# consensus-shipyard/ipc-filecoin-proofs

Hardware: AMD Instinct MI355X
Metric: Merkle proofs verified/sec + HBM GB/s, 1M-receipt synthetic tipset, 1/2/4/8 GPU (higher is better)
Workload: dtype u64; 1 GPU; BASELINE.json configs[2] (the 1M-receipt tipset the metric is quoted on): 1000000 receipts (Amtv0<Receipt> + one Amt<...; receipts_per_gpu=1000000, claims_per_gpu=1000000, witness_blocks_per_gpu=1288038, witness_bytes_per_gpu=439923915, scan_matches=1002, device=AMD Radeon Graphics

## Files before the change

ipc-filecoin-proofs_amd/csrc/kernels/verify_dev.h:

```cpp
#pragma once
#include "claims_dev.h"
#include "event_table.h"
#include "amt_enum.h"
#include "event_table.h"
#include "tipset_ctx.h"
#include "types_dev.h"

namespace ipcfp {


constexpr unsigned long long kEmptySlot64 = ~0ULL;

__device__ __forceinline__ uint32_t exec_find(const unsigned long long* slots, uint32_t mask, const CidKey* keys,
                                              const CidKey& key) {
    const uint64_t h = cid_hash64(key);
    uint32_t s = uint32_t(h >> 32) & mask;
    for (;;) {
        const unsigned long long cur = slots[s];
        if (cur == kEmptySlot64) return kNoBlock;
        if (uint32_t(cur >> 32) == uint32_t(h) && cid_equal(keys[uint32_t(cur)], key)) return uint32_t(cur);
        s = (s + 1) & mask;
    }
}

__device__ __forceinline__ bool ev_trusted(const ipcfp_trust_policy_t& t, long long epoch) {
    if (t.kind == 0) return true;
    if (t.ec_chain_empty) return false;
    return epoch >= t.min_epoch && epoch <= t.max_epoch;
}

__device__ __forceinline__ bool bytes_equal_global(const uint8_t* __restrict__ a, const uint8_t* __restrict__ b, uint32_t n) {
    uint64_t diff = 0;
    uint32_t i = 0;
    typedef unsigned long long u64x2_t __attribute__((ext_vector_type(2)));
    for (; i + 16 <= n; i += 16) {
        u64x2_t x, y;
        __builtin_memcpy(&x, a + i, 16);
        __builtin_memcpy(&y, b + i, 16);
        diff |= (x.x ^ y.x) | (x.y ^ y.y);
    }
    for (; i + 8 <= n; i += 8) {
        uint64_t x, y;
        __builtin_memcpy(&x, a + i, 8);
        __builtin_memcpy(&y, b + i, 8);
        diff |= x ^ y;
    }
    for (; i < n; ++i) diff |= uint64_t(a[i] ^ b[i]);
    return diff == 0;
}

__device__ __forceinline__ uint32_t verify_event_record(const WitnessView& w, const EventClaimPacked& c, const EventRec& e,
                                                        const uint8_t* __restrict__ blob, const ipcfp_event_filter_t& filter,
                                                        bool has_filter) {
    if (e.emitter != c.emitter) return IPCFP_ST_FALSE_EMITTER;
    if (!(e.base_flags & kEvIsLog)) return IPCFP_ST_FALSE_NOT_EVM_LOG;
    const uint32_t nt = uint32_t(e.base_flags >> kEvTopicShift) & 0xffu;
    if (nt != c.n_topics) return IPCFP_ST_FALSE_TOPIC_COUNT;
    const uint8_t* item = w.arena + (e.base_flags & kEvBaseMask);
    const bool case_a = (e.base_flags & kEvCaseA) != 0;
    for (uint32_t i = 0; i < nt; ++i) {
        const uint8_t* claimed = blob + c.topics_off + 33u * i;
        if (!claimed[0]) return IPCFP_ST_FALSE_TOPIC;
        const uint32_t rel = case_a ? uint32_t(e.topic_rel[0]) + 32u * i : uint32_t(e.topic_rel[i & 3u]);
        if (!bytes_equal_global(item + rel, claimed + 1, 32)) return IPCFP_ST_FALSE_TOPIC;
    }
    if (!(c.flags & EC_DATA_MATCHABLE) || c.data_len != e.data_len) return IPCFP_ST_FALSE_DATA;
    if (!bytes_equal_global(item + e.data_rel, blob + c.data_off, c.data_len)) return IPCFP_ST_FALSE_DATA;
    if (has_filter) {
        if (nt < 2) return IPCFP_ST_FALSE_FILTER;
        const uint32_t r1 = case_a ? uint32_t(e.topic_rel[0]) + 32u : uint32_t(e.topic_rel[1]);
        if (!bytes_equal_global(item + e.topic_rel[0], filter.topic0, 32) || !bytes_equal_global(item + r1, filter.topic1, 32))
            return IPCFP_ST_FALSE_FILTER;
    }
    return IPCFP_ST_TRUE;
}

__device__ __forceinline__ uint32_t verify_event_prefix(const EventClaimPacked& c, const TipsetCtxDev& tc,
                                                        const ipcfp_trust_policy_t& trust) {
    if (!(tc.flags & TC_PARENTS_PARSED) || !(tc.flags & TC_CHILD_PARSED)) return IPCFP_ST_ERR_BAD_CLAIM;
    if (!ev_trusted(trust, c.parent_epoch)) return IPCFP_ST_FALSE_UNTRUSTED_PARENT;
    if (!ev_trusted(trust, c.child_epoch)) return IPCFP_ST_FALSE_UNTRUSTED_CHILD;
    if (tc.child_status != IPCFP_ST_TRUE) return tc.child_status;
    if (!tc.parents_match) return IPCFP_ST_FALSE_PARENTS_MISMATCH;
    if (tc.child_height != c.child_epoch) return IPCFP_ST_FALSE_CHILD_EPOCH;
    if (tc.n_parents == 0) return IPCFP_ST_ERR_EMPTY_PARENTS;
    if (tc.parent0_status != IPCFP_ST_TRUE) return tc.parent0_status;
    if (tc.parent0_height != c.parent_epoch) return IPCFP_ST_FALSE_PARENT_EPOCH;
    if (tc.exec_status != IPCFP_ST_TRUE) return tc.exec_status;
    if (!(c.flags & EC_MSG_PARSED)) return IPCFP_ST_ERR_BAD_CLAIM;
    if (tc.exec_inv && c.exec_index < tc.exec_len && cid_equal(tc.exec_keys[tc.exec_inv[c.exec_index]], c.message))
        return IPCFP_ST_TRUE;
    const uint32_t raw = tc.exec_slots ? exec_find(tc.exec_slots, tc.exec_mask, tc.exec_keys, c.message) : kNoBlock;
    if (raw == kNoBlock) return IPCFP_ST_FALSE_MSG_NOT_IN_EXEC;
    if (uint64_t(tc.exec_pos[raw]) != c.exec_index) return IPCFP_ST_FALSE_EXEC_INDEX;
    return IPCFP_ST_TRUE;
}

struct EventCtxFacts {
    uint32_t flags, n_parents, child_status, parents_match, parent0_status, exec_status;
    long long child_height, parent0_height;
    const CidKey* exec_keys;
    const uint32_t* exec_inv;
    uint64_t exec_len;
    bool has_receipt_table;
    uint64_t n_receipt_leaves, receipt_first;
    const ReceiptRec* receipt_recs;
    const EventRec* event_recs;
};

__device__ __forceinline__ EventCtxFacts event_ctx_facts(const TipsetCtxDev& tc) {
    return EventCtxFacts{tc.flags,        tc.n_parents,      tc.child_status, tc.parents_match,
                         tc.parent0_status, tc.exec_status,  tc.child_height, tc.parent0_height,
                         tc.exec_keys,    tc.exec_inv,       tc.exec_len,     tc.receipt_leaves != nullptr && tc.receipt_recs != nullptr,
                         tc.n_receipt_leaves, tc.receipt_first, tc.receipt_recs, tc.event_recs};
}

struct Verdict {
    uint32_t st = IPCFP_ST_TRUE;
    bool settled = false;
    __device__ __forceinline__ void rung(bool fails, uint32_t status) {
        st = (!settled && fails) ? status : st;
        settled = settled || fails;
    }
};

__device__ __forceinline__ void event_prefix_rungs(Verdict& v, const EventClaimPacked& c, const EventCtxFacts& f,
                                                   const ipcfp_trust_policy_t& trust) {
    v.rung(!(f.flags & TC_PARENTS_PARSED) || !(f.flags & TC_CHILD_PARSED), IPCFP_ST_ERR_BAD_CLAIM);
    v.rung(!ev_trusted(trust, c.parent_epoch), IPCFP_ST_FALSE_UNTRUSTED_PARENT);
    v.rung(!ev_trusted(trust, c.child_epoch), IPCFP_ST_FALSE_UNTRUSTED_CHILD);
    v.rung(f.child_status != IPCFP_ST_TRUE, f.child_status);
    v.rung(!f.parents_match, IPCFP_ST_FALSE_PARENTS_MISMATCH);
    v.rung(f.child_height != c.child_epoch, IPCFP_ST_FALSE_CHILD_EPOCH);
    v.rung(f.n_parents == 0, IPCFP_ST_ERR_EMPTY_PARENTS);
    v.rung(f.parent0_status != IPCFP_ST_TRUE, f.parent0_status);
    v.rung(f.parent0_height != c.parent_epoch, IPCFP_ST_FALSE_PARENT_EPOCH);
    v.rung(f.exec_status != IPCFP_ST_TRUE, f.exec_status);
    v.rung(!(c.flags & EC_MSG_PARSED), IPCFP_ST_ERR_BAD_CLAIM);
}

__device__ __forceinline__ uint32_t verify_event_from_table(const WitnessView& w, const EventClaimPacked& c,
                                                            const TipsetCtxDev& tc, const uint8_t* __restrict__ blob,
                                                            const ipcfp_event_filter_t& filter, bool has_filter,
                                                            ValueLoc* where, bool& settled) {
    settled = false;
    if (!tc.receipt_leaves || !tc.receipt_recs || c.exec_index < tc.receipt_first ||
        c.exec_index - tc.receipt_first >= tc.n_receipt_leaves)
        return kStPending;
    const ReceiptRec rr = tc.receipt_recs[c.exec_index - tc.receipt_first];
    if (rr.kind == RK_WALK) return kStPending;
    settled = true;
    if (rr.kind == RK_NO_EVENTS) return IPCFP_ST_FALSE_NO_EVENTS_ROOT;
    if (rr.kind >= 64) return rr.kind;
    if (c.event_index == ~0ULL) return IPCFP_ST_ERR;
    if (c.event_index >= 64 || !((rr.bitmap >> c.event_index) & 1ull)) return IPCFP_ST_FALSE_NO_EVENT;
    const EventRec e = tc.event_recs[rr.first + __popcll(rr.bitmap & ((1ull << c.event_index) - 1ull))];
    if (where) *where = ValueLoc{rr.block, uint32_t((e.base_flags & kEvBaseMask) - w.off[rr.block]), e.ev_len};
    return verify_event_record(w, c, e, blob, filter, has_filter);
}

__device__ __forceinline__ bool claim_in_bounds(const EventClaimPacked& c, uint32_t n_ctxs, uint64_t blob_len) {
    return c.context < n_ctxs && c.n_topics <= (1u << 20) && uint64_t(c.topics_off) + 33ull * c.n_topics <= blob_len &&
           uint64_t(c.data_off) + c.data_len <= blob_len;
}

}
```

ipc-filecoin-proofs_amd/csrc/kernels/verify_table.hip:

```cpp
#include <hip/hip_runtime.h>

#include <cstddef>

#include "../common.h"
#include "launch.h"
#include "verify_dev.h"

namespace ipcfp {

typedef unsigned long long u64x2_t __attribute__((ext_vector_type(2)));

__device__ __forceinline__ u64x2_t ld16(const uint8_t* __restrict__ p) {
    u64x2_t v;
    __builtin_memcpy(&v, p, 16);
    return v;
}
__device__ __forceinline__ bool differ32(const u64x2_t a[2], const u64x2_t b[2]) {
    return (((a[0].x ^ b[0].x) | (a[0].y ^ b[0].y)) | ((a[1].x ^ b[1].x) | (a[1].y ^ b[1].y))) != 0;
}

struct ClaimedBytes {
    u64x2_t topic[2][2];
    uint32_t flag[2];
    u64x2_t data[2];
};

__device__ __forceinline__ void load_claimed(const EventClaimPacked& c, const uint8_t* __restrict__ blob, ClaimedBytes& p) {
    p = ClaimedBytes{};
    if (c.n_topics >= 1 && c.n_topics <= 2) {
        const uint8_t* q = blob + c.topics_off;
        p.flag[0] = q[0];
        p.topic[0][0] = ld16(q + 1);
        p.topic[0][1] = ld16(q + 17);
        if (c.n_topics == 2) {
            p.flag[1] = q[33];
            p.topic[1][0] = ld16(q + 34);
            p.topic[1][1] = ld16(q + 50);
        }
    }
    if ((c.flags & EC_DATA_MATCHABLE) && c.data_len == 32) {
        p.data[0] = ld16(blob + c.data_off);
        p.data[1] = ld16(blob + c.data_off + 16);
    }
}

__device__ __forceinline__ uint32_t verify_event_record_batched(const WitnessView& w, const EventClaimPacked& c, const EventRec& e,
                                                                const ClaimedBytes& p, const uint8_t* __restrict__ blob,
                                                                const ipcfp_event_filter_t& filter, bool has_filter) {
    if (e.emitter != c.emitter) return IPCFP_ST_FALSE_EMITTER;
    if (!(e.base_flags & kEvIsLog)) return IPCFP_ST_FALSE_NOT_EVM_LOG;
    const uint32_t nt = uint32_t(e.base_flags >> kEvTopicShift) & 0xffu;
    if (nt != c.n_topics) return IPCFP_ST_FALSE_TOPIC_COUNT;
    if (nt > 2) return verify_event_record(w, c, e, blob, filter, has_filter);
    const uint8_t* item = w.arena + (e.base_flags & kEvBaseMask);
    const bool case_a = (e.base_flags & kEvCaseA) != 0;
    const uint32_t rel0 = e.topic_rel[0], rel1 = case_a ? uint32_t(e.topic_rel[0]) + 32u : uint32_t(e.topic_rel[1]);
    const bool data_shape = (c.flags & EC_DATA_MATCHABLE) && c.data_len == e.data_len;
    const bool data_batched = data_shape && c.data_len == 32;
    u64x2_t t0[2] = {}, t1[2] = {}, d[2] = {};
    if (nt >= 1) {
        t0[0] = ld16(item + rel0);
        t0[1] = ld16(item + rel0 + 16);
    }
    if (nt == 2) {
        t1[0] = ld16(item + rel1);
        t1[1] = ld16(item + rel1 + 16);
    }
    if (data_batched) {
        d[0] = ld16(item + e.data_rel);
        d[1] = ld16(item + e.data_rel + 16);
    }
    if (nt >= 1 && (!p.flag[0] || differ32(p.topic[0], t0))) return IPCFP_ST_FALSE_TOPIC;
    if (nt == 2 && (!p.flag[1] || differ32(p.topic[1], t1))) return IPCFP_ST_FALSE_TOPIC;
    if (!data_shape) return IPCFP_ST_FALSE_DATA;
    if (data_batched ? differ32(p.data, d) : !bytes_equal_global(item + e.data_rel, blob + c.data_off, c.data_len))
        return IPCFP_ST_FALSE_DATA;
    if (has_filter) {
        if (nt < 2) return IPCFP_ST_FALSE_FILTER;
        u64x2_t f0[2], f1[2];
        __builtin_memcpy(f0, filter.topic0, 32);
        __builtin_memcpy(f1, filter.topic1, 32);
        if (differ32(t0, f0) || differ32(t1, f1)) return IPCFP_ST_FALSE_FILTER;
    }
    return IPCFP_ST_TRUE;
}

__device__ __forceinline__ uint32_t verify_table_one(const WitnessView& w, const EventClaimPacked& c, const TipsetCtxDev& tc,
                                                     const uint8_t* __restrict__ blob, const ipcfp_trust_policy_t& trust,
                                                     const ipcfp_event_filter_t& filter, bool has_filter, ValueLoc* where) {
    ClaimedBytes p;
    load_claimed(c, blob, p);
    const bool tabulated = tc.receipt_leaves && tc.receipt_recs && c.exec_index >= tc.receipt_first &&
                           c.exec_index - tc.receipt_first < tc.n_receipt_leaves;
    ReceiptRec rr{RK_WALK, 0, 0, kNoBlock, 0};
    if (tabulated) rr = tc.receipt_recs[c.exec_index - tc.receipt_first];
    const uint32_t st = verify_event_prefix(c, tc, trust);
    if (st != IPCFP_ST_TRUE) return st;
    if (!tabulated || rr.kind == RK_WALK) return kStPending;
    if (rr.kind == RK_NO_EVENTS) return IPCFP_ST_FALSE_NO_EVENTS_ROOT;
    if (rr.kind >= 64) return rr.kind;
    if (c.event_index == ~0ULL) return IPCFP_ST_ERR;
    if (c.event_index >= 64 || !((rr.bitmap >> c.event_index) & 1ull)) return IPCFP_ST_FALSE_NO_EVENT;
    const EventRec e = tc.event_recs[rr.first + __popcll(rr.bitmap & ((1ull << c.event_index) - 1ull))];
    if (where) *where = ValueLoc{rr.block, uint32_t((e.base_flags & kEvBaseMask) - w.off[rr.block]), e.ev_len};
    return verify_event_record_batched(w, c, e, p, blob, filter, has_filter);
}

typedef const __attribute__((address_space(1))) uint8_t* gbytes_t;
__device__ __forceinline__ gbytes_t guarded(bool ok, const void* p, const void* safe) {
    return ok ? (gbytes_t)p : (gbytes_t)safe;
}
__device__ __forceinline__ u64x2_t ld16(gbytes_t p) {
    u64x2_t v;
    __builtin_memcpy(&v, p, 16);
    return v;
}
__device__ __forceinline__ void batch_end(uint64_t a, uint64_t b = 0, uint64_t c = 0, uint64_t d = 0, uint64_t e = 0) {
    asm volatile("" ::"v"(a), "v"(b), "v"(c), "v"(d), "v"(e));
}

static_assert(offsetof(ReceiptRec, first) == 4 && offsetof(ReceiptRec, bitmap) == 8 && offsetof(ReceiptRec, block) == 16,
              "verify_table_hot reads a ReceiptRec as three words");
static_assert(offsetof(EventRec, topic_rel) == 16 && offsetof(EventRec, data_rel) == 24 && offsetof(EventRec, ev_len) == 26 &&
                  offsetof(EventRec, data_len) == 28,
              "verify_table_hot reads an EventRec as four words");

__device__ __forceinline__ bool hot_shape(const EventClaimPacked& c) {
    return c.n_topics <= 2 && (!(c.flags & EC_DATA_MATCHABLE) || c.data_len == 32);
}

__device__ __forceinline__ uint32_t verify_table_hot(const WitnessView& w, const EventClaimPacked& c, const TipsetCtxDev& tc,
                                                     const uint8_t* __restrict__ blob, const ipcfp_trust_policy_t& trust,
                                                     const ipcfp_event_filter_t& filter, bool has_filter, bool want_where,
                                                     const void* safe, ValueLoc& loc, bool& cold) {
    const EventCtxFacts f = event_ctx_facts(tc);
    Verdict v;
    event_prefix_rungs(v, c, f, trust);
    const bool pre_ok = !v.settled;
    const bool tabulated = f.has_receipt_table && c.exec_index >= f.receipt_first && c.exec_index - f.receipt_first < f.n_receipt_leaves;
    uint64_t rw[3];
    __builtin_memcpy(rw, guarded(tabulated, f.receipt_recs + (c.exec_index - f.receipt_first), safe), 24);
    const bool inv_ok = pre_ok && f.exec_inv && f.exec_keys && c.exec_index < f.exec_len;
    uint32_t inv;
    __builtin_memcpy(&inv, guarded(inv_ok, f.exec_inv + c.exec_index, safe), 4);
    const bool matchable = (c.flags & EC_DATA_MATCHABLE) != 0;
    const gbytes_t q0 = guarded(c.n_topics >= 1, blob + c.topics_off, safe);
    const gbytes_t q1 = guarded(c.n_topics == 2, blob + c.topics_off + 33, safe);
    const gbytes_t qd = guarded(matchable, blob + c.data_off, safe);
    ClaimedBytes p;
    p.flag[0] = q0[0];
    p.topic[0][0] = ld16(q0 + 1);
    p.topic[0][1] = ld16(q0 + 17);
    p.flag[1] = q1[0];
    p.topic[1][0] = ld16(q1 + 1);
    p.topic[1][1] = ld16(q1 + 17);
    p.data[0] = ld16(qd);
    p.data[1] = ld16(qd + 16);
    batch_end(rw[0], rw[1], rw[2], inv);
    const uint32_t rr_kind = uint32_t(rw[0]), rr_first = uint32_t(rw[0] >> 32), rr_block = uint32_t(rw[2]);
    const uint64_t rr_bitmap = rw[1];

    CidKey key;
    __builtin_memcpy(&key, guarded(inv_ok, f.exec_keys + inv, safe), 40);
    const uint32_t bit = uint32_t(c.event_index) & 63u;
    const bool present = c.event_index < 64 && ((rr_bitmap >> bit) & 1ull);
    const bool have_event = pre_ok && tabulated && rr_kind == RK_TABLE && f.event_recs && present;
    const uint32_t slot = rr_first + uint32_t(__popcll(rr_bitmap & ((1ull << bit) - 1ull)));
    uint64_t ew[4];
    __builtin_memcpy(ew, guarded(have_event, f.event_recs + slot, safe), 32);
    uint64_t block_off;
    __builtin_memcpy(&block_off, guarded(want_where && have_event, w.off + rr_block, safe), 8);
    batch_end(key.w[0], key.w[1], key.w[2], key.w[3], key.w[4]);
    batch_end(ew[0], ew[1], ew[2], ew[3], block_off);

    const bool exec_ok = inv_ok && cid_equal(key, c.message);
    v.rung(!tabulated || rr_kind == RK_WALK, kStPending);
    v.rung(rr_kind == RK_NO_EVENTS, IPCFP_ST_FALSE_NO_EVENTS_ROOT);
    v.rung(rr_kind >= 64, rr_kind);
    v.rung(c.event_index == ~0ULL, IPCFP_ST_ERR);
    v.rung(!present, IPCFP_ST_FALSE_NO_EVENT);
    const bool reached = !v.settled;
    cold = pre_ok && (!exec_ok || (reached && !have_event));

    const uint64_t base_flags = ew[0], e_emitter = ew[1];
    const uint32_t rel0 = uint32_t(ew[2]) & 0xffffu, rel1_b = uint32_t(ew[2] >> 16) & 0xffffu;
    const uint32_t data_rel = uint32_t(ew[3]) & 0xffffu, ev_len = uint32_t(ew[3] >> 16) & 0xffffu, e_data_len = uint32_t(ew[3] >> 32);
    v.rung(e_emitter != c.emitter, IPCFP_ST_FALSE_EMITTER);
    v.rung(!(base_flags & kEvIsLog), IPCFP_ST_FALSE_NOT_EVM_LOG);
    const uint32_t nt = uint32_t(base_flags >> kEvTopicShift) & 0xffu;
    v.rung(nt != c.n_topics, IPCFP_ST_FALSE_TOPIC_COUNT);

    const bool bytes_wanted = have_event && exec_ok && !v.settled;
    const uint8_t* item = w.arena + (base_flags & kEvBaseMask);
    const uint32_t rel1 = (base_flags & kEvCaseA) ? rel0 + 32u : rel1_b;
    const bool data_shape = matchable && c.data_len == e_data_len;
    const gbytes_t a0 = guarded(bytes_wanted && nt >= 1, item + rel0, safe);
    const gbytes_t a1 = guarded(bytes_wanted && nt == 2, item + rel1, safe);
    const gbytes_t ad = guarded(bytes_wanted && data_shape, item + data_rel, safe);
    const u64x2_t t0[2] = {ld16(a0), ld16(a0 + 16)}, t1[2] = {ld16(a1), ld16(a1 + 16)}, d[2] = {ld16(ad), ld16(ad + 16)};

    v.rung(nt >= 1 && (!p.flag[0] || differ32(p.topic[0], t0)), IPCFP_ST_FALSE_TOPIC);
    v.rung(nt == 2 && (!p.flag[1] || differ32(p.topic[1], t1)), IPCFP_ST_FALSE_TOPIC);
    v.rung(!data_shape, IPCFP_ST_FALSE_DATA);
    v.rung(differ32(p.data, d), IPCFP_ST_FALSE_DATA);
    u64x2_t f0[2], f1[2];
    __builtin_memcpy(f0, filter.topic0, 32);
    __builtin_memcpy(f1, filter.topic1, 32);
    v.rung(has_filter && nt < 2, IPCFP_ST_FALSE_FILTER);
    v.rung(has_filter && (differ32(t0, f0) || differ32(t1, f1)), IPCFP_ST_FALSE_FILTER);

    const bool located = reached && have_event;
    loc.block = located ? rr_block : kNoBlock;
    loc.off = located ? uint32_t((base_flags & kEvBaseMask) - block_off) : 0u;
    loc.len = located ? ev_len : 0u;
    return v.st;
}

__global__ __launch_bounds__(256) void k_verify_events_table(WitnessView w, const EventClaimPacked* __restrict__ claims, uint32_t n,
                                                             const TipsetCtxDev* __restrict__ ctxs, uint32_t n_ctxs,
                                                             const uint8_t* __restrict__ blob, uint64_t blob_len,
                                                             ipcfp_trust_policy_t trust, ipcfp_event_filter_t filter,
                                                             int has_filter, uint8_t* __restrict__ status,
                                                             ValueLoc* __restrict__ where) {
    const uint32_t t = blockIdx.x * blockDim.x + threadIdx.x;
    const bool live = t < n;
    EventClaimPacked c;
    if (live) c = claims[t];
    else c.context = 0;
    ValueLoc loc{kNoBlock, 0, 0};
    uint32_t st = IPCFP_ST_ERR_BAD_CLAIM;
    const bool inb = live && claim_in_bounds(c, n_ctxs, blob_len);
    const uint32_t ctx0 = __builtin_amdgcn_readfirstlane(inb ? c.context : 0xffffffffu);
    bool cold = inb;
    if (ctx0 != 0xffffffffu && __all(!inb || c.context == ctx0)) {
        if (inb && hot_shape(c)) {
            ValueLoc hot_loc;
            bool again;
            const uint32_t hot_st = verify_table_hot(w, c, ctxs[ctx0], blob, trust, filter, has_filter != 0, where != nullptr,
                                                     claims + t, hot_loc, again);
            st = again ? st : hot_st;
            loc.block = again ? loc.block : hot_loc.block;
            loc.off = again ? loc.off : hot_loc.off;
            loc.len = again ? loc.len : hot_loc.len;
            cold = again;
        }
    }
    if (__any(cold)) {
        if (cold) {
            const EventClaimPacked* mine = claims + t;
            asm volatile("" : "+v"(mine));
            const EventClaimPacked cc = *mine;
            ValueLoc cold_loc{kNoBlock, 0, 0};
            st = verify_table_one(w, cc, ctxs[cc.context], blob, trust, filter, has_filter != 0, &cold_loc);
            loc = cold_loc;
        }
    }
    if (!live) return;
    status[t] = uint8_t(st);
    if (where) where[t] = loc;
}

int launch_verify_events_table(ipcfp_ctx* ctx, const WitnessView& w, const EventClaimPacked* claims_d, uint32_t n,
                               const TipsetCtxDev* ctxs_d, uint32_t n_ctxs, const uint8_t* blob_d, uint64_t blob_len,
                               const ipcfp_trust_policy_t& trust, const ipcfp_event_filter_t& filter, int has_filter,
                               uint8_t* status_d, void* where_d) {
    if (n == 0) return IPCFP_OK;
    hipLaunchKernelGGL(k_verify_events_table, dim3(div_up(n, 256)), dim3(256), 0, ctx->stream, w, claims_d, n, ctxs_d, n_ctxs,
                       blob_d, blob_len, trust, filter, has_filter, status_d, static_cast<ValueLoc*>(where_d));
    IPCFP_HIP(ctx, hipGetLastError());
    return IPCFP_OK;
}

}
```

Baseline: 1.268 billion proofs/s.

## Stage claims and claimed blob window through LDS with coalesced wave-wide copies

The table-verify kernel now copies each wave's claim structs into a per-wave shared-memory region with coalesced 16-byte loads. It then computes the wave's min/max span of claimed topic/data bytes in the blob and stages that window into LDS before doing per-lane unaligned reads via alignbyte. The goal is to replace scattered per-lane global loads with contiguous wave-wide transfers. The cost is a larger LDS footprint per block (about 26KB), extra wave barriers, and a fallback to direct global loads when the window is too large. A small change also packs topic_rel into a 64-bit value to avoid dynamic indexing.

```diff
diff --git a/ipc-filecoin-proofs_amd/csrc/kernels/verify_dev.h b/ipc-filecoin-proofs_amd/csrc/kernels/verify_dev.h
--- a/ipc-filecoin-proofs_amd/csrc/kernels/verify_dev.h
+++ b/ipc-filecoin-proofs_amd/csrc/kernels/verify_dev.h
@@ -58,10 +58,12 @@
     if (nt != c.n_topics) return IPCFP_ST_FALSE_TOPIC_COUNT;
     const uint8_t* item = w.arena + (e.base_flags & kEvBaseMask);
     const bool case_a = (e.base_flags & kEvCaseA) != 0;
+    const uint64_t rels = uint64_t(e.topic_rel[0]) | uint64_t(e.topic_rel[1]) << 16 | uint64_t(e.topic_rel[2]) << 32 |
+                          uint64_t(e.topic_rel[3]) << 48;
     for (uint32_t i = 0; i < nt; ++i) {
         const uint8_t* claimed = blob + c.topics_off + 33u * i;
         if (!claimed[0]) return IPCFP_ST_FALSE_TOPIC;
-        const uint32_t rel = case_a ? uint32_t(e.topic_rel[0]) + 32u * i : uint32_t(e.topic_rel[i & 3u]);
+        const uint32_t rel = case_a ? uint32_t(e.topic_rel[0]) + 32u * i : uint32_t(rels >> (16u * (i & 3u))) & 0xffffu;
         if (!bytes_equal_global(item + rel, claimed + 1, 32)) return IPCFP_ST_FALSE_TOPIC;
     }
     if (!(c.flags & EC_DATA_MATCHABLE) || c.data_len != e.data_len) return IPCFP_ST_FALSE_DATA;
diff --git a/ipc-filecoin-proofs_amd/csrc/kernels/verify_table.hip b/ipc-filecoin-proofs_amd/csrc/kernels/verify_table.hip
--- a/ipc-filecoin-proofs_amd/csrc/kernels/verify_table.hip
+++ b/ipc-filecoin-proofs_amd/csrc/kernels/verify_table.hip
@@ -5,6 +5,7 @@
 #include "../common.h"
 #include "launch.h"
 #include "verify_dev.h"
+#include "verify_window.h"
 
 namespace ipcfp {
 
@@ -129,33 +130,98 @@
     return c.n_topics <= 2 && (!(c.flags & EC_DATA_MATCHABLE) || c.data_len == 32);
 }
 
-__device__ __forceinline__ uint32_t verify_table_hot(const WitnessView& w, const EventClaimPacked& c, const TipsetCtxDev& tc,
-                                                     const uint8_t* __restrict__ blob, const ipcfp_trust_policy_t& trust,
-                                                     const ipcfp_event_filter_t& filter, bool has_filter, bool want_where,
-                                                     const void* safe, ValueLoc& loc, bool& cold) {
+constexpr uint32_t kStageStride = kVerifyWindowBytes + 16u;
+constexpr uint32_t kStageLoads = (kVerifyWindowBytes + 1023u) / 1024u;
+
+__device__ __forceinline__ void stage_copy(uint8_t* __restrict__ region, const uint8_t* __restrict__ src, uint32_t bytes, uint32_t lane) {
+    const uint32_t whole = bytes & ~15u;
+    u64x2_t v[kStageLoads];
+#pragma unroll
+    for (uint32_t k = 0; k < kStageLoads; ++k) {
+        const uint32_t o = (k * 64u + lane) * 16u;
+        v[k] = u64x2_t{0, 0};
+        if (o < whole) v[k] = ld16(src + o);
+    }
+#pragma unroll
+    for (uint32_t k = 0; k < kStageLoads; ++k) {
+        const uint32_t o = (k * 64u + lane) * 16u;
+        if (o < whole) __builtin_memcpy(__builtin_assume_aligned(region + o, 16), &v[k], 16);
+    }
+    if (whole + lane < bytes) region[whole + lane] = src[whole + lane];
+}
+__device__ __forceinline__ void stage_publish() {
+    __builtin_amdgcn_fence(__ATOMIC_RELEASE, "wavefront");
+    __builtin_amdgcn_wave_barrier();
+    __builtin_amdgcn_fence(__ATOMIC_ACQUIRE, "wavefront");
+}
+__device__ __forceinline__ void region_ld32(const uint8_t* region, uint32_t j, u64x2_t out[2]) {
+    const uint8_t* p = static_cast<const uint8_t*>(__builtin_assume_aligned(region + (j & ~3u), 4));
+    const uint32_t s = j & 3u;
+    uint32_t x[9], a[8];
+#pragma unroll
+    for (int i = 0; i < 9; ++i) __builtin_memcpy(&x[i], p + 4 * i, 4);
+#pragma unroll
+    for (int i = 0; i < 8; ++i) a[i] = __builtin_amdgcn_alignbyte(x[i + 1], x[i], s);
+    out[0] = u64x2_t{a[0] | uint64_t(a[1]) << 32, a[2] | uint64_t(a[3]) << 32};
+    out[1] = u64x2_t{a[4] | uint64_t(a[5]) << 32, a[6] | uint64_t(a[7]) << 32};
+}
+__device__ __forceinline__ uint32_t wave_min(uint32_t v) {
+#pragma unroll
+    for (int m = 32; m >= 1; m >>= 1) v = min(v, uint32_t(__shfl_xor(v, m, 64)));
+    return v;
+}
+__device__ __forceinline__ uint32_t wave_max(uint32_t v) {
+#pragma unroll
+    for (int m = 32; m >= 1; m >>= 1) v = max(v, uint32_t(__shfl_xor(v, m, 64)));
+    return v;
+}
+
+__device__ __forceinline__ uint32_t verify_table_hot(const WitnessView& w, const EventClaimPacked& c, bool hot, const TipsetCtxDev& tc,
+                                                     const uint8_t* __restrict__ blob, uint64_t blob_len,
+                                                     const ipcfp_trust_policy_t& trust, const ipcfp_event_filter_t& filter,
+                                                     bool has_filter, bool want_where, const void* safe, uint8_t* region,
+                                                     uint32_t lane, ValueLoc& loc, bool& cold) {
     const EventCtxFacts f = event_ctx_facts(tc);
     Verdict v;
     event_prefix_rungs(v, c, f, trust);
-    const bool pre_ok = !v.settled;
-    const bool tabulated = f.has_receipt_table && c.exec_index >= f.receipt_first && c.exec_index - f.receipt_first < f.n_receipt_leaves;
+    const bool pre_ok = hot && !v.settled;
+    const bool tabulated = hot && f.has_receipt_table && c.exec_index >= f.receipt_first && c.exec_index - f.receipt_first < f.n_receipt_leaves;
     uint64_t rw[3];
     __builtin_memcpy(rw, guarded(tabulated, f.receipt_recs + (c.exec_index - f.receipt_first), safe), 24);
     const bool inv_ok = pre_ok && f.exec_inv && f.exec_keys && c.exec_index < f.exec_len;
     uint32_t inv;
     __builtin_memcpy(&inv, guarded(inv_ok, f.exec_inv + c.exec_index, safe), 4);
     const bool matchable = (c.flags & EC_DATA_MATCHABLE) != 0;
-    const gbytes_t q0 = guarded(c.n_topics >= 1, blob + c.topics_off, safe);
-    const gbytes_t q1 = guarded(c.n_topics == 2, blob + c.topics_off + 33, safe);
-    const gbytes_t qd = guarded(matchable, blob + c.data_off, safe);
+    const bool rd0 = hot && c.n_topics >= 1, rd1 = hot && c.n_topics == 2, rdd = hot && matchable;
+    uint64_t lo, hi;
+    const bool reads = verify_window_lane(hot ? c.n_topics : 0u, c.topics_off, rdd, c.data_off, lo, hi);
+    const uint64_t start = verify_window_start(wave_min(reads ? uint32_t(lo) : 0xffffffffu));
+    const uint32_t win_len = __builtin_amdgcn_readfirstlane(
+        __any(reads) ? verify_window_len(start, wave_max(reads ? verify_window_rel_end(hi, start) : 0u), blob_len) : 0u);
     ClaimedBytes p;
-    p.flag[0] = q0[0];
-    p.topic[0][0] = ld16(q0 + 1);
-    p.topic[0][1] = ld16(q0 + 17);
-    p.flag[1] = q1[0];
-    p.topic[1][0] = ld16(q1 + 1);
-    p.topic[1][1] = ld16(q1 + 17);
-    p.data[0] = ld16(qd);
-    p.data[1] = ld16(qd + 16);
+    if (win_len) {
+        stage_copy(region, blob + start, win_len, lane);
+        stage_publish();
+        const uint32_t j0 = rd0 ? uint32_t(c.topics_off - start) : 0u, j1 = rd1 ? j0 + 33u : 0u;
+        const uint32_t jd = rdd ? uint32_t(c.data_off - start) : 0u;
+        p.flag[0] = region[j0];
+        region_ld32(region, j0 + (rd0 ? 1u : 0u), p.topic[0]);
+        p.flag[1] = region[j1];
+        region_ld32(region, j1 + (rd1 ? 1u : 0u), p.topic[1]);
+        region_ld32(region, jd, p.data);
+    } else {
+        const gbytes_t q0 = guarded(rd0, blob + c.topics_off, safe);
+        const gbytes_t q1 = guarded(rd1, blob + c.topics_off + 33, safe);
+        const gbytes_t qd = guarded(rdd, blob + c.data_off, safe);
+        p.flag[0] = q0[0];
+        p.topic[0][0] = ld16(q0 + 1);
+        p.topic[0][1] = ld16(q0 + 17);
+        p.flag[1] = q1[0];
+        p.topic[1][0] = ld16(q1 + 1);
+        p.topic[1][1] = ld16(q1 + 17);
+        p.data[0] = ld16(qd);
+        p.data[1] = ld16(qd + 16);
+    }
     batch_end(rw[0], rw[1], rw[2], inv);
     const uint32_t rr_kind = uint32_t(rw[0]), rr_first = uint32_t(rw[0] >> 32), rr_block = uint32_t(rw[2]);
     const uint64_t rr_bitmap = rw[1];
@@ -168,8 +234,8 @@
     const uint32_t slot = rr_first + uint32_t(__popcll(rr_bitmap & ((1ull << bit) - 1ull)));
     uint64_t ew[4];
     __builtin_memcpy(ew, guarded(have_event, f.event_recs + slot, safe), 32);
-    uint64_t block_off;
-    __builtin_memcpy(&block_off, guarded(want_where && have_event, w.off + rr_block, safe), 8);
+    uint64_t block_off = 0;
+    if (want_where) __builtin_memcpy(&block_off, guarded(have_event, w.off + rr_block, safe), 8);
     batch_end(key.w[0], key.w[1], key.w[2], key.w[3], key.w[4]);
     batch_end(ew[0], ew[1], ew[2], ew[3], block_off);
 
@@ -222,27 +288,35 @@
                                                              ipcfp_trust_policy_t trust, ipcfp_event_filter_t filter,
                                                              int has_filter, uint8_t* __restrict__ status,
                                                              ValueLoc* __restrict__ where) {
+    __shared__ __attribute__((aligned(16))) uint8_t regions[4][kStageStride];
     const uint32_t t = blockIdx.x * blockDim.x + threadIdx.x;
+    const uint32_t lane = threadIdx.x & 63u, first = t - lane;
+    if (first >= n) return;
     const bool live = t < n;
-    EventClaimPacked c;
-    if (live) c = claims[t];
-    else c.context = 0;
+    uint8_t* const region = regions[threadIdx.x >> 6];
+    stage_copy(region, reinterpret_cast<const uint8_t*>(claims + first), min(64u, n - first) * uint32_t(sizeof(EventClaimPacked)), lane);
+    stage_publish();
+    EventClaimPacked c{};
+    if (live) __builtin_memcpy(&c, __builtin_assume_aligned(region + lane * sizeof(EventClaimPacked), 8), sizeof c);
+    stage_publish();
     ValueLoc loc{kNoBlock, 0, 0};
     uint32_t st = IPCFP_ST_ERR_BAD_CLAIM;
     const bool inb = live && claim_in_bounds(c, n_ctxs, blob_len);
     const uint32_t ctx0 = __builtin_amdgcn_readfirstlane(inb ? c.context : 0xffffffffu);
     bool cold = inb;
     if (ctx0 != 0xffffffffu && __all(!inb || c.context == ctx0)) {
-        if (inb && hot_shape(c)) {
+        const bool hot = inb && hot_shape(c);
+        if (__any(hot)) {
             ValueLoc hot_loc;
             bool again;
-            const uint32_t hot_st = verify_table_hot(w, c, ctxs[ctx0], blob, trust, filter, has_filter != 0, where != nullptr,
-                                                     claims + t, hot_loc, again);
-            st = again ? st : hot_st;
-            loc.block = again ? loc.block : hot_loc.block;
-            loc.off = again ? loc.off : hot_loc.off;
-            loc.len = again ? loc.len : hot_loc.len;
-            cold = again;
+            const uint32_t hot_st = verify_table_hot(w, c, hot, ctxs[ctx0], blob, blob_len, trust, filter, has_filter != 0,
+                                                     where != nullptr, claims + first, region, lane, hot_loc, again);
+            const bool keep = !hot || again;
+            st = keep ? st : hot_st;
+            loc.block = keep ? loc.block : hot_loc.block;
+            loc.off = keep ? loc.off : hot_loc.off;
+            loc.len = keep ? loc.len : hot_loc.len;
+            cold = hot ? again : cold;
         }
     }
     if (__any(cold)) {
diff --git a/ipc-filecoin-proofs_amd/csrc/kernels/verify_window.h b/ipc-filecoin-proofs_amd/csrc/kernels/verify_window.h
--- /dev/null
+++ b/ipc-filecoin-proofs_amd/csrc/kernels/verify_window.h
@@ -0,0 +1,46 @@
+#pragma once
+#include <cstdint>
+
+#if defined(__HIPCC__)
+#define IPCFP_WINDOW_FN __host__ __device__ inline
+#else
+#define IPCFP_WINDOW_FN inline
+#endif
+
+namespace ipcfp {
+
+constexpr uint32_t kVerifyWindowBytes = 64u * 104u;
+
+IPCFP_WINDOW_FN bool verify_window_lane(uint32_t n_topics, uint32_t topics_off, bool data_read, uint32_t data_off, uint64_t& lo,
+                                        uint64_t& hi) {
+    lo = ~0ull;
+    hi = 0;
+    if (n_topics >= 1) {
+        lo = topics_off;
+        hi = uint64_t(topics_off) + 33ull * n_topics;
+    }
+    if (data_read) {
+        const uint64_t a = data_off, b = a + 32ull;
+        lo = a < lo ? a : lo;
+        hi = b > hi ? b : hi;
+    }
+    return hi != 0;
+}
+
+IPCFP_WINDOW_FN uint64_t verify_window_start(uint64_t lo_min) { return lo_min & ~15ull; }
+
+IPCFP_WINDOW_FN uint32_t verify_window_rel_end(uint64_t hi, uint64_t start) {
+    const uint64_t d = hi - start;
+    return d > kVerifyWindowBytes ? kVerifyWindowBytes + 1u : uint32_t(d);
+}
+
+IPCFP_WINDOW_FN uint32_t verify_window_len(uint64_t start, uint32_t rel_end_max, uint64_t blob_len) {
+    if (rel_end_max == 0 || rel_end_max > kVerifyWindowBytes) return 0;
+    uint64_t end = (start + rel_end_max + 15ull) & ~15ull;
+    end = end > blob_len ? blob_len : end;
+    if (end < start + rel_end_max) return 0;
+    const uint64_t len = end - start;
+    return len > kVerifyWindowBytes ? 0u : uint32_t(len);
+}
+
+}
```

After: 1.289 billion proofs/s (median of 6 runs). 1.7% higher.
